# CliMA/CloudMicrophysics.jl

Hardware: AMD Instinct MI355X
Metric: grid-points/sec SB2006 2M tendency sweep (higher is better)
Workload: dtype f32

## Files before the change

cloudmicrophysics.jl_amd/csrc/cmx_sb2006.hpp:

```cpp
#pragma once
#include <cmath>
#include <cstdint>

#include "../../include/cmx.h"
#include "cmx_math.hpp"

namespace cmx {

enum : int { VEL_NONE = 0, VEL_SB = 1, VEL_CHEN = 2, VEL_CHEN_GEN = 3 };

template <typename FT> struct SbConsts {
    FT T_0, LH_v0, dcp, R_v, inv_R_v;
    FT ps_c0, ps_a, ps_b, inv_T_tr;
    FT cp_d, cpm_qt, cpm_ql;
    FT tau_ce;
    FT inv_K, Rv_over_D, eps_1m;
    FT xr_min, xr_max, N0_min, N0_max, lam_min, lam_max, pi_rho_w;
    FT l2_6xstar, l2_Drc;
    FT l2_pi_rho_w, l2_xr_min, l2_xr_max, l2_N0_min, l2_N0_max, l2_lam_min, l2_lam_max, inv_eps_1m;
    FT ga_c1, ga_e1, ga_c2, ga_e2;
    FT gb_c1, gb_e1, gb_c2, gb_e2;
    FT a_vent_1, bSc_vent_1;
    FT sqrt_alpha_nu, beta, ev_rho0_q;
    FT sqrt_alpha_nu_rho0q;
// ... 197 lines not shown
    vt_n = FT(0);
    vt_m = FT(0);
    if constexpr (VEL == VEL_SB) {
        const FT Dr_mean = M::exp2_fin(-l2_lam);
        FT pa0 = FT(1), pb0 = FT(1), pa1 = FT(1), pb1 = FT(1);
        if constexpr (!LIMITED) {
            const FT lam = M::exp2_fin(l2_lam);
            const FT ta = c.rc2 * lam, tb = c.rc2 * (lam + c.cR);
            pa0 = M::exp2_fin(ta * FT(-1.4426950408889634));
            pb0 = pa0 * c.e_rc2cR;
            pa1 = (((ta + FT(3)) * ta + FT(6)) * ta + FT(6)) * pa0 * FT(1.0 / 6.0);
            pb1 = (((tb + FT(3)) * tb + FT(6)) * tb + FT(6)) * pb0 * FT(1.0 / 6.0);
        }
        const FT s = c.vel_s * rs_rho;
        const FT inv_d1 = M::rcp_nz(M::fma(c.cR, Dr_mean, FT(1)));
        const FT inv_d2 = inv_d1 * inv_d1;
        const FT vt0 = M::max(FT(0), s * (c.aR * pa0 - c.bR * pb0 * inv_d1));
        const FT vt1 = M::max(FT(0), s * (c.aR * pa1 - c.bR * pb1 * (inv_d2 * inv_d2)));
        vt_n = no_N_rai ? FT(0) : vt0;
        vt_m = no_q_rai ? FT(0) : vt1;
    } else if constexpr (VEL == VEL_CHEN) {
        const FT lam = M::exp2_fin(l2_lam);
        const FT rho_c = M::max(rho, FT(0));
        const FT t = rho_c - FT(0.5 * kChenGammaRhoMax);
        const FT l2_lam4 = FT(4) * l2_lam;
        FT vt0 = FT(0), vt3 = FT(0);
#pragma unroll
        for (int i = 0; i < 3; ++i) {
            const FT l2_den = M::log2(lam + c.ch_c1000[i]);
            FT L0 = chen_log_eval<S>(c.chl, 0, i, t), L3 = chen_log_eval<S>(c.chl, 1, i, t);
            if (i == 2) { const FT ar = c.ch_a3_pow * M::log2(rho_c); L0 += ar; L3 += ar; }
            const FT e0 = M::exp2(M::fma(-M::fma(-c.ch_b_rho, rho_c, c.chl.b1[i]), l2_den, L0 + l2_lam));
            const FT e3 = M::exp2(M::fma(-M::fma(-c.ch_b_rho, rho_c, c.chl.b4[i]), l2_den, L3 + l2_lam4));
            vt0 = M::fma(c.chl.sgn[i], e0, vt0);
            vt3 = M::fma(c.chl.sgn[i], e3, vt3);
        }
        vt0 = M::max(FT(0), vt0);
        vt3 = M::max(FT(0), vt3);
        {
            const typename M::Mask beyond = rho_c > FT(kChenGammaRhoMax);
            vt0 = beyond ? M::nan() : vt0;
            vt3 = beyond ? M::nan() : vt3;
        }
        vt_n = no_N_rai ? FT(0) : vt0;
        vt_m = no_q_rai ? FT(0) : vt3;
    } else if constexpr (VEL == VEL_CHEN_GEN) {
        const FT lam = M::exp2_fin(l2_lam);
        const FT rho_c = M::max(rho, FT(0));
        const FT l2_q = c.ch_rho0_l2e * rho_c;
        const FT l2_rho = M::log2(rho_c);
        const FT l2_lam_inv = -l2_lam;
        FT vt0 = FT(0), vt3 = FT(0);
#pragma unroll
        for (int i = 0; i < 3; ++i) {
            const FT bi = M::fma(-c.ch_b_rho, rho_c, c.ch_b[i]);
            FT l2_mag = l2_q + bi * c.l2_1000 + (i == 2 ? c.ch_a3_pow * l2_rho : FT(0));
            const FT l2_den = M::log2(lam + c.ch_c1000[i]);
            const FT g1 = tgamma_general<FT>(bi + FT(1));
            const FT e0 = M::exp2(l2_mag - l2_lam_inv - (bi + FT(1)) * l2_den);
            const FT e3 = M::exp2(l2_mag - FT(4) * l2_lam_inv - (bi + FT(4)) * l2_den);
            vt0 = M::fma(c.ch_a[i] * e0, g1, vt0);
            const FT g4 = g1 * (bi + FT(3)) * (bi + FT(2)) * (bi + FT(1)) * FT(1.0 / 6.0);
            vt3 = M::fma(c.ch_a[i] * e3, g4, vt3);
        }
        vt0 = M::max(FT(0), vt0);
        vt3 = M::max(FT(0), vt3);
        vt_n = no_N_rai ? FT(0) : vt0;
        vt_m = no_q_rai ? FT(0) : vt3;
    }
}

template <typename FT, typename CH> inline int chen_vel_kind(const CH &ch) {
    ChenLog<FT> g;
    return make_chen_log<FT>(ch, g) ? VEL_CHEN : VEL_CHEN_GEN;
}

template <typename WR> inline bool sb_integer_exponents(const WR &wr) {
    const auto &sb = wr.seifert_beheng;
    return sb.acnv.b == 3 && sb.accr.c == 4 && sb.self.d == -5;
}
template <typename FT, bool LIMITED, int VEL, bool ICE = false, bool INTPOW = false, typename C>
__device__ __forceinline__ SbRates<FT> sb2006_point(const C &c0, FT rho, FT T, FT q_tot,
                                                    FT q_lcl, FT q_rai, FT N_lcl, FT N_rai,
                                                    FT n_lcl, FT n_rai, FT q_ice = FT(0), FT cpm_qi = FT(0)) {
    using M = Math<FT>;
    const FT eps = FT(M::eps());
    SbRates<FT> r;

    const FT rs_rho = M::rsqrt(rho);
    const FT inv_rho = rs_rho * rs_rho;
    r.inv_rho = inv_rho;

    const C &c = c0;
    const FT inv_T = M::rcp_nz(T);
    const FT L_v = M::fma(c.dcp, T - c.T_0, c.LH_v0);
    const FT l2_ps = M::fma(c.ps_a, M::log2(T * c.inv_T_tr), M::fma(c.ps_b, c.inv_T_tr - inv_T, c.ps_c0));
    const FT p_sat = M::exp2_fin(l2_ps);
    const FT q_liq = q_lcl + q_rai;
    FT q_vap = M::max(FT(0), q_tot - q_liq);
    if constexpr (ICE) q_vap = M::max(FT(0), (q_tot - q_liq) - q_ice);
    const FT rho_RvT = rho * (c.R_v * T);
    const FT inv_p_sat = M::rcp(p_sat);
    const FT inv_RvT = c.inv_R_v * inv_T;
    const FT q_sat = p_sat * (inv_rho * inv_RvT);
    const FT LoRT = L_v * inv_RvT;
    {
        FT cp_air = M::fma(c.cpm_ql, q_liq, M::fma(c.cpm_qt, q_tot, c.cp_d));
        if constexpr (ICE) cp_air = M::fma(cpm_qi, q_ice, cp_air);
        const FT dqsl_dT = q_sat * (LoRT * inv_T - inv_T);
        const FT excess = q_vap - q_sat;
        const FT inv_ts = cp_air * M::rcp_nz(c.tau_ce * M::fma(L_v, dqsl_dT, cp_air));
        const FT evap_lim = -M::min(-excess, M::max(FT(0), q_lcl));
        r.cond = (excess < FT(0) ? evap_lim : excess) * inv_ts;
    }
    const FT S = M::fma(q_vap * rho_RvT, inv_p_sat, FT(-1));
    const FT inv_p_safe = M::min(inv_p_sat, c.inv_eps_1m);
    const FT G = M::rcp_nz(M::fma(L_v * c.inv_K * inv_T, LoRT - FT(1), c.Rv_over_D * T * inv_p_safe));

    const FT sq_lcl = M::max(q_lcl, eps);
    const FT sN_lcl = M::max(N_lcl, eps);
    const FT sq_rai = M::max(q_rai, eps);
    const FT sN_rai = M::max(N_rai, eps);
    const FT L_lcl = rho * sq_lcl;
    const FT L_rai = rho * sq_rai;
    const FT x_lcl_raw = L_lcl * M::rcp_nz(sN_lcl);
    using B = typename M::Mask;
    const B no_q_lcl = q_lcl < eps, no_N_lcl = N_lcl < eps, no_q_rai = q_rai < eps;
    const FT inv_qsum = M::rcp_nz(sq_lcl + sq_rai);
    const FT tau = sq_rai * inv_qsum;
    const FT one_m_tau = sq_lcl * inv_qsum;
    const FT l2_tau = M::log2(tau);
    {
        const C &c = consts_after(c0, G);
        const FT x_lcl = M::min(c.x_star, x_lcl_raw);
        const FT tau_a = M::exp2_fin(c.acnv_a * l2_tau);
        FT pow_b;
        if constexpr (INTPOW) { const FT u = FT(1) - tau_a; pow_b = u * u * u; }
        else pow_b = M::exp2(c.acnv_b * M::log2(FT(1) - tau_a));
        const FT phi_raw = keep(c.acnv_A * tau_a * pow_b);
        const FT phi_au = no_q_rai ? FT(0) : phi_raw;
        const FT u = (L_lcl * x_lcl) * c.sqrt_kfac;
        const FT inv_omt = M::rcp_nz(one_m_tau);
        const FT dL_rai = (u * u) * M::fma(phi_au, inv_omt * inv_omt, FT(1)) * (c.acnv_rho0 * inv_rho);
        const FT dN_rai = dL_rai * c.inv_x_star;
        const B gate = m_or(no_q_lcl, no_N_lcl);
        r.au_dq_rai = gate ? FT(0) : dL_rai * inv_rho;
        r.au_dq_lcl = -r.au_dq_rai;
        r.au_dN_rai = gate ? FT(0) : dN_rai;
        r.au_dN_lcl = FT(-2) * r.au_dN_rai;
    }
    {
        const C &c = consts_after(c0, G);
        const FT Lr = rho * q_lcl;
        const FT sc = -c.ksc * inv_rho * (Lr * Lr) - r.au_dN_lcl;
        r.lsc = no_q_lcl ? FT(0) : sc;
        r.lsc_plus_au = no_q_lcl ? FT(0) : -c.ksc * inv_rho * (Lr * Lr);
    }
    {
        const C &c = consts_after(c0, G);
        FT pow_c;
        if constexpr (INTPOW) { const FT t = tau * M::rcp_nz(tau + c.tau_0), t2 = t * t; pow_c = t2 * t2; }
        else pow_c = M::exp2_fin(c.accr_c * (l2_tau - M::log2(tau + c.tau_0)));
        const FT phi_ac = keep(pow_c);
        const FT k_ac = c.kcr_s * rs_rho * L_rai * phi_ac;
        const FT dq = keep(k_ac * L_lcl * inv_rho);
        const FT dN = keep(-k_ac * sN_lcl);
        const B gate = m_or(no_q_lcl, no_q_rai, no_N_lcl);
        r.ac_dq_rai = gate ? FT(0) : dq;
        r.ac_dq_lcl = -r.ac_dq_rai;
        r.ac_dN_lcl = gate ? FT(0) : dN;
    }

    const C &c_psd = consts_after(c0, r.ac_dN_lcl);
    const SbRainPsd<FT> psd = sb2006_rain_psd<FT, LIMITED>(c_psd, L_rai, sN_rai);
    const FT l2_xr = psd.l2_xr, l2_lam = psd.l2_lam;
    const FT l2_Dr = (l2_xr + c_psd.l2_Drc) * FT(1.0 / 3.0);
    const FT Dr = M::exp2_fin(l2_Dr);
    const B no_N_rai = N_rai < eps;
    {
        const C &c = consts_after(c0, r.ac_dN_lcl);
        FT pw;
        if constexpr (INTPOW) { const FT r1 = M::rcp_nz(M::fma(c.kappa_rr_K, Dr, FT(1))), r2 = r1 * r1; pw = r2 * r2 * r1; }
        else pw = M::exp2_fin(c.self_d * M::log2(M::fma(c.kappa_rr_K, Dr, FT(1))));
        const FT sc = -c.krr_s * rs_rho * N_rai * L_rai * pw;
        const B gate = m_or(no_q_rai, no_N_rai);
        r.rsc = gate ? FT(0) : sc;
        const FT dD = Dr - c.Deq;
        const FT br_lin = keep(c.kbr * dD), br_exp = keep(M::exp2_fin(c.kappa_br_l2e * dD) - FT(1));
        const FT phi_br = (Dr < c.Dr_th) ? FT(-1) : ((Dr <= c.Deq) ? br_lin : br_exp);
        r.rbr = gate ? FT(0) : -(phi_br + FT(1)) * r.rsc;
    }
    {
        const C &c = consts_after(c0, r.rbr);
        const FT l2_t = (c.l2_6xstar - l2_xr) * FT(1.0 / 3.0);
        FT t_star;
        if constexpr (M::IS_F64) t_star = c.tstar_Dr * M::rcp_nz(Dr);
        else t_star = M::exp2_fin(l2_t);
        const FT e_tx = M::exp2_fin(M::fma(t_star, FT(-1.4426950408889634), -l2_xr));
        const FT g_a = M::rcp_nz(M::fma(c.ga_c1, M::exp2_fin(c.ga_e1 * l2_t), c.ga_c2 * M::exp2_fin(c.ga_e2 * l2_t)));
        const FT g_b = M::rcp(M::fma(c.gb_c1, M::exp2_fin(c.gb_e1 * l2_t), c.gb_c2 * M::exp2_fin(c.gb_e2 * l2_t)));
        const FT sqrt_N_Re = c.sqrt_alpha_nu_rho0q * M::sqrt_pos(rs_rho) *
                             M::exp2_fin(FT(0.5) * M::fma(c.beta, l2_xr, l2_Dr));
        const FT Fv0 = M::fma(g_b, sqrt_N_Re, g_a);
        const FT Fv1 = M::fma(c.bSc_vent_1, sqrt_N_Re, c.a_vent_1);
        const FT common = c.two_pi * G * S * N_rai * Dr;
        const FT dN = M::min(FT(0), common * Fv0 * e_tx);
        const FT dq = M::min(FT(0), common * Fv1 * inv_rho);
        const B gate_q = m_or(no_q_rai, N_rai <= eps, S >= FT(0));
        const B gate_N = m_or(gate_q, l2_xr < c.l2_gate_N);
        r.evN = gate_N ? FT(0) : dN;
        r.evq = gate_q ? FT(0) : dq;
    }
    {
        const C &c = consts_after(c0, r.evq);
        const FT tl = no_q_lcl ? FT(0) : clampv(n_lcl, q_lcl * c.inv_xc_max, q_lcl * c.inv_xc_min);
        r.na_lcl = (tl - n_lcl) * c.inv_tau_na;
        const FT tr = no_q_rai ? FT(0) : clampv(n_rai, q_rai * c.inv_xr_max, q_rai * c.inv_xr_min);
        r.na_rai = (tr - n_rai) * c.inv_tau_na;
    }
    sb2006_rain_velocity<FT, LIMITED, VEL>(consts_after(c0, r.evq), rho, rs_rho, l2_lam, no_N_rai, no_q_rai, r.vt_n, r.vt_m);
    return r;
}

}
```

cloudmicrophysics.jl_amd/csrc/cmx_sb2006_kernels.hip:

```cpp
#include <hip/hip_runtime.h>

#include <algorithm>
#include <type_traits>

#include "cmx_sb2006_kernels.hpp"

namespace cmx {

static int decode_vel(uint32_t flags, bool want) {
    if (!want) return VEL_NONE;
    const bool sb = flags & CMX_VEL_SB2006, ch = flags & CMX_VEL_CHEN2022;
    if (sb == ch) return -1;
    return sb ? VEL_SB : VEL_CHEN;
}

#ifndef CMX_TEND_BS
#define CMX_TEND_BS 128
#endif
constexpr int kTendBS = CMX_TEND_BS;

template <typename FT, typename WR, typename TH, typename VL>
static int32_t tendencies_entry(const WR *wr, const TH *tps, const VL *vel, uint32_t flags, int64_t n, const FT *rho,
                                const FT *T, const FT *q_tot, const FT *q_lcl, const FT *n_lcl, const FT *q_rai,
                                const FT *n_rai, FT *dq_lcl, FT *dn_lcl, FT *dq_rai, FT *dn_rai, FT *vt_n, FT *vt_m,
                                void *stream) {
    if (!wr || !tps) return CMX_ERR_BAD_ARG;
    CMX_TRY_COUNT(n);
    if (!rho || !T || !q_tot || !q_lcl || !n_lcl || !q_rai || !n_rai || !dq_lcl || !dn_lcl || !dq_rai || !dn_rai)
        return CMX_ERR_BAD_ARG;
    const bool want_vel = vt_n || vt_m;
    int velk = decode_vel(flags, want_vel);
    if (velk < 0 || (want_vel && !vel)) return CMX_ERR_BAD_ARG;
    if (velk == VEL_CHEN) velk = chen_vel_kind<FT>(vel->chen2022);
    const bool limited = flags & CMX_SB2006_LIMITED;
    if ((flags & CMX_SB2006_LIMITED) && !sb_limiters_ok(*wr)) return CMX_ERR_BAD_ARG;
    if (velk == VEL_SB && !sb_rain_vel_ok(*vel, limited)) return CMX_ERR_BAD_ARG;
    const SbConsts<FT> c = make_sb_consts<FT>(*wr, *tps, vel, (double)Math<FT>::eps_1m());
    const bool intpow = sb_integer_exponents(*wr);
    bool known = true;
    hipStream_t s = reinterpret_cast<hipStream_t>(stream);
    constexpr int VEC = sizeof(FT) == 8 ? 1 : Math<FT>::VEC;
    const void *ptrs[] = {rho, T, q_tot, q_lcl, n_lcl, q_rai, n_rai, dq_lcl, dn_lcl, dq_rai, dn_rai, vt_n, vt_m};
    for_each_range<FT, VEC>(ptrs, n, [&](auto vec_tag, int64_t lo, int64_t count) {
        constexpr int V = decltype(vec_tag)::value;
        SbIn<FT> in{rho + lo, T + lo, q_tot + lo, q_lcl + lo, n_lcl + lo, q_rai + lo, n_rai + lo};
        SbOut<FT> out{dq_lcl + lo, dn_lcl + lo, dq_rai + lo, dn_rai + lo, shift(vt_n, lo), shift(vt_m, lo)};
        const int64_t nvec = count / V;
        known &= dispatch([&](auto L, auto K, auto I) {
            launch<kTendBS>(sb2006_tendencies_kernel<FT, decltype(L)::value, decltype(K)::value, V, kTendBS, 1, true, decltype(I)::value>, nvec, s, c, in, out, nvec);
        }, flag(limited), one_of<VEL_NONE, VEL_SB, VEL_CHEN, VEL_CHEN_GEN>(velk), flag(intpow));
    });
    if (!known) return CMX_ERR_BAD_ARG;
    return launched();
}

template <typename FT, typename WR, typename TH>
static int32_t fields_entry(const WR *wr, const TH *tps, uint32_t flags, int64_t n_seg, int64_t seg_len, const FT *const *in,
                            const int64_t *in_stride, FT *const *out, const int64_t *out_stride, FT *aos, void *stream) {
    if (!wr || !tps || (flags & ~(uint32_t)CMX_SB2006_LIMITED)) return CMX_ERR_BAD_ARG;
    if ((flags & CMX_SB2006_LIMITED) && !sb_limiters_ok(*wr)) return CMX_ERR_BAD_ARG;
    const SbConsts<FT> c = make_sb_consts<FT>(*wr, *tps, (const std::conditional_t<std::is_same_v<FT, float>, cmx_rain_vel_f32, cmx_rain_vel_f64> *)nullptr,
                                              (double)Math<FT>::eps_1m());
    hipStream_t s = reinterpret_cast<hipStream_t>(stream);
    return dispatch_or((int32_t)CMX_ERR_BAD_ARG, [&](auto L, auto I) {
        return launch_layout<FT, Sb2006LayoutPolicy<FT, decltype(L)::value, decltype(I)::value>>(c, n_seg, seg_len, in, in_stride, out, out_stride, aos, s);
    }, flag(flags & CMX_SB2006_LIMITED), flag(sb_integer_exponents(*wr)));
}

template <typename FT, typename WR, typename TH, typename VL>
static int32_t process_entry(const WR *wr, const TH *tps, const VL *vel, uint32_t flags, int64_t n, const FT *q_tot,
                             const FT *q_lcl, const FT *q_rai, const FT *N_lcl, const FT *N_rai, const FT *rho,
                             const FT *T, FT *const out[CMX_SB2006_NPROC], void *stream) {
    if (!wr || !tps || !out) return CMX_ERR_BAD_ARG;
    CMX_TRY_COUNT(n);
    if (!q_tot || !q_lcl || !q_rai || !N_lcl || !N_rai || !rho || !T) return CMX_ERR_BAD_ARG;
    const bool want_vel = out[CMX_SB_RAI_VEL_N] || out[CMX_SB_RAI_VEL_M];
    int velk = decode_vel(flags, want_vel);
    if (velk < 0 || (want_vel && !vel)) return CMX_ERR_BAD_ARG;
    if (velk == VEL_CHEN) velk = chen_vel_kind<FT>(vel->chen2022);
    const bool limited = flags & CMX_SB2006_LIMITED;
    if ((flags & CMX_SB2006_LIMITED) && !sb_limiters_ok(*wr)) return CMX_ERR_BAD_ARG;
    if (velk == VEL_SB && !sb_rain_vel_ok(*vel, limited)) return CMX_ERR_BAD_ARG;
    const SbConsts<FT> c = make_sb_consts<FT>(*wr, *tps, vel, (double)Math<FT>::eps_1m());
    SbProcOut<FT> o;
    for (int k = 0; k < CMX_SB2006_NPROC; ++k) o.col[k] = out[k];
    hipStream_t s = reinterpret_cast<hipStream_t>(stream);
    const dim3 grid(grid_for(n));
    if (!dispatch([&](auto L, auto K) {
            launch_grid(sb2006_process_kernel<FT, decltype(L)::value, decltype(K)::value>, grid, dim3(kBlock), 0, s, c, q_tot, q_lcl, q_rai, N_lcl, N_rai, rho, T, o, n);
        }, flag(limited), one_of<VEL_NONE, VEL_SB, VEL_CHEN, VEL_CHEN_GEN>(velk)))
        return CMX_ERR_BAD_ARG;
    return launched();
}

template <typename FT>
__global__ __launch_bounds__(kBlock) void sb2006_cloud_velocity_kernel(const CloudVelConsts<FT> c, const FT *__restrict__ q_liq,
                                                                       const FT *__restrict__ rho, const FT *__restrict__ N_liq,
                                                                       FT *__restrict__ vt_n, FT *__restrict__ vt_m, const int64_t n) {
    Math<FT>::prepare();
    const int64_t i = (int64_t)blockIdx.x * kBlock + threadIdx.x;
    if (i >= n) return;
    FT v0, v1;
    sb2006_cloud_velocity(c, q_liq[i], rho[i], N_liq[i], v0, v1);
    if (vt_n) vt_n[i] = v0;
    if (vt_m) vt_m[i] = v1;
}

template <typename FT, typename PDF, typename VEL>
static int32_t cloud_velocity_entry(const PDF *pdf, const VEL *vel, int64_t n, const FT *q_liq, const FT *rho, const FT *N_liq, FT *vt_n,
                                    FT *vt_m, void *stream) {
    if (!pdf || !vel) return CMX_ERR_BAD_ARG;
    CMX_TRY_COUNT(n);
    if (!q_liq || !rho || !N_liq) return CMX_ERR_BAD_ARG;
    const CloudVelConsts<FT> c = make_cloud_vel_consts<FT>(*pdf, *vel);
    launch<kBlock>(sb2006_cloud_velocity_kernel<FT>, n, reinterpret_cast<hipStream_t>(stream), c, q_liq, rho, N_liq, vt_n, vt_m, n);
    return launched();
}

template <typename FT> struct Bulk2mConsts {
    uint32_t scheme; FT eps_1m, eps_m;
    FT kk_l2A, kk_a, kk_b, kk_c, kk_accr_A, kk_accr_a, kk_accr_b;
    FT b_l2C, b_a, b_b, b_c, b_N_0, b_d_low, b_d_high, b_k, b_accr_A;
    FT t_a, t_b, t_D, t_thr_c, t_k, t_accr_A;
    FT l_rvol_c, l_E_0, l_R_6C_0, l_k;
};
template <typename FT> __device__ __forceinline__ FT logistic_dev(FT x, FT x_0, FT k, FT eps) {
    using M = Math<FT>;
    x = M::max(FT(0), x);
    const FT xs = M::max(x, eps), x0s = M::max(x_0, eps);
    const FT z = k * (xs * M::rcp(x0s) - x0s * M::rcp(xs));
    const FT r = M::rcp(FT(1) + M::exp2(-z * FT(1.4426950408889634)));
    return x < eps ? FT(0) : (x_0 < eps ? FT(1) : r);
}
template <typename FT>
__global__ __launch_bounds__(kBlock) void bulk_2m_cloud_to_rain_kernel(const Bulk2mConsts<FT> c, const FT *__restrict__ q_lcl,
                                                                       const FT *__restrict__ q_rai, const FT *__restrict__ rho,
                                                                       const FT *__restrict__ N_d, FT *__restrict__ acnv,
                                                                       FT *__restrict__ accr, const int64_t n) {
    Math<FT>::prepare();
    using M = Math<FT>;
    const int64_t i = (int64_t)blockIdx.x * kBlock + threadIdx.x;
    if (i >= n) return;
    const uint32_t sch = c.scheme & 0xffu;
    const bool smooth = c.scheme & CMX_2M_SMOOTH_TRANSITION;
    const FT ql_raw = q_lcl[i], r = rho[i];
    const FT ql = M::max(FT(0), ql_raw);
    if (acnv) {
        const FT Nd = N_d[i];
        const FT l2q = M::log2(ql), l2N = M::log2(Nd), l2r = M::log2(r);
        FT v;
        if (sch == CMX_2M_KK2000) {
            v = M::exp2(c.kk_l2A + c.kk_a * l2q + c.kk_b * l2N + c.kk_c * l2r);
        } else if (sch == CMX_2M_B1994) {
            FT d;
            if (smooth) {
                const FT f = logistic_dev<FT>(Nd, c.b_N_0, c.b_k, c.eps_1m);
                d = f * c.b_d_low + (FT(1) - f) * c.b_d_high;
            } else {
                d = Nd >= c.b_N_0 ? c.b_d_low : c.b_d_high;
            }
            v = M::exp2(c.b_l2C + c.b_a * M::log2(d) + c.b_b * (l2q + l2r) + c.b_c * l2N - l2r);
        } else if (sch == CMX_2M_TC1980) {
            const FT thr = c.t_thr_c * Nd * M::rcp(r);
            const FT out = smooth ? logistic_dev<FT>(ql, thr, c.t_k, c.eps_1m) : (ql - thr > FT(0) ? FT(1) : FT(0));
            v = c.t_D * M::exp2(c.t_a * l2q + c.t_b * l2N) * out;
        } else {
            const FT l2_rv3 = M::log2(c.l_rvol_c * ql_raw * r * M::rcp(Nd));
            const FT r_vol = M::exp2(l2_rv3 * FT(1.0 / 3.0));
            const FT l2_b6 = FT(1.0 / 3.0) * M::log2((r_vol + FT(3)) * M::rcp(r_vol));
            const FT R_6 = M::exp2(l2_b6) * r_vol;
            const FT l2_qr = M::log2(ql_raw * r);
            const FT R_6C = c.l_R_6C_0 * M::exp2(FT(-1.0 / 6.0) * l2_qr) * M::rsqrt(R_6);
            const FT out = smooth ? logistic_dev<FT>(R_6, R_6C, c.l_k, c.eps_1m) : (R_6 - R_6C > FT(0) ? FT(1) : FT(0));
            const FT val = c.l_E_0 * M::exp2(FT(6) * l2_b6 + FT(3) * l2_qr - l2N - l2r) * out;
            v = ql_raw <= c.eps_m ? FT(0) : val;
        }
        acnv[i] = v;
    }
    if (accr) {
        const FT qr = M::max(FT(0), q_rai[i]);
        FT v;
        if (sch == CMX_2M_KK2000) v = c.kk_accr_A * M::exp2(c.kk_accr_a * M::log2(ql * qr) + c.kk_accr_b * M::log2(r));
        else if (sch == CMX_2M_B1994) v = c.b_accr_A * ql * r * qr;
        else v = c.t_accr_A * ql * qr;
        accr[i] = v;
    }
}

template <typename FT, typename SC>
static int32_t bulk_2m_entry(const SC *p, uint32_t scheme, int64_t n, const FT *q_lcl, const FT *q_rai, const FT *rho, const FT *N_d,
                             FT *acnv, FT *accr, void *stream) {
    const uint32_t sch = scheme & 0xffu;
    if (!p || sch > CMX_2M_LD2004 || (scheme & ~(0xffu | CMX_2M_SMOOTH_TRANSITION))) return CMX_ERR_BAD_ARG;
    CMX_TRY_COUNT_LIMIT(n);
    if (sch == CMX_2M_LD2004 && accr) return CMX_ERR_BAD_ARG;
    if (n == 0) return CMX_OK;
    if (!q_lcl || !rho || (acnv && !N_d) || (accr && !q_rai) || (!acnv && !accr)) return CMX_ERR_BAD_ARG;
    const double pi = 3.14159265358979323846;
    Bulk2mConsts<FT> c{};
    c.scheme = scheme; c.eps_1m = Math<FT>::eps_1m(); c.eps_m = Math<FT>::eps();
    c.kk_l2A = (FT)std::log2((double)p->kk2000.acnv_A); c.kk_a = p->kk2000.acnv_a; c.kk_b = p->kk2000.acnv_b; c.kk_c = p->kk2000.acnv_c;
    c.kk_accr_A = p->kk2000.accr_A; c.kk_accr_a = p->kk2000.accr_a; c.kk_accr_b = p->kk2000.accr_b;
    c.b_l2C = (FT)std::log2((double)p->b1994.acnv_C); c.b_a = p->b1994.acnv_a; c.b_b = p->b1994.acnv_b; c.b_c = p->b1994.acnv_c;
    c.b_N_0 = p->b1994.acnv_N_0; c.b_d_low = p->b1994.acnv_d_low; c.b_d_high = p->b1994.acnv_d_high; c.b_k = p->b1994.acnv_k;
    c.b_accr_A = p->b1994.accr_A;
    c.t_a = p->tc1980.acnv_a; c.t_b = p->tc1980.acnv_b; c.t_D = p->tc1980.acnv_D; c.t_k = p->tc1980.acnv_k; c.t_accr_A = p->tc1980.accr_A;
    c.t_thr_c = (FT)((double)p->tc1980.acnv_m0_liq_coeff * std::pow((double)p->tc1980.acnv_r_0, (double)p->tc1980.acnv_me_liq));
    c.l_rvol_c = (FT)(3.0 / 4.0 / pi / (double)p->ld2004.rho_w * 1e18);
    c.l_E_0 = p->ld2004.E_0; c.l_R_6C_0 = p->ld2004.R_6C_0; c.l_k = p->ld2004.k;
    launch<kBlock>(bulk_2m_cloud_to_rain_kernel<FT>, n, reinterpret_cast<hipStream_t>(stream), c, q_lcl, q_rai, rho, N_d, acnv, accr, n);
    return launched();
}

}

extern "C" {

int32_t cmx_bulk_2m_cloud_to_rain_f32(const cmx_bulk_2m_schemes_f32 *schemes, uint32_t scheme, int64_t n, const float *q_lcl,
                                      const float *q_rai, const float *rho, const float *N_d, float *acnv, float *accr, void *stream) {
    return cmx::bulk_2m_entry<float>(schemes, scheme, n, q_lcl, q_rai, rho, N_d, acnv, accr, stream);
}
int32_t cmx_bulk_2m_cloud_to_rain_f64(const cmx_bulk_2m_schemes_f64 *schemes, uint32_t scheme, int64_t n, const double *q_lcl,
                                      const double *q_rai, const double *rho, const double *N_d, double *acnv, double *accr,
                                      void *stream) {
    return cmx::bulk_2m_entry<double>(schemes, scheme, n, q_lcl, q_rai, rho, N_d, acnv, accr, stream);
}

int32_t cmx_sb2006_cloud_terminal_velocity_f32(const cmx_cloud_pdf_sb2006_f32 *pdf_c, const cmx_stokes_vel_f32 *vel, int64_t n,
                                               const float *q_liq, const float *rho, const float *N_liq, float *vt_n, float *vt_m,
                                               void *stream) {
    return cmx::cloud_velocity_entry<float>(pdf_c, vel, n, q_liq, rho, N_liq, vt_n, vt_m, stream);
}
int32_t cmx_sb2006_cloud_terminal_velocity_f64(const cmx_cloud_pdf_sb2006_f64 *pdf_c, const cmx_stokes_vel_f64 *vel, int64_t n,
                                               const double *q_liq, const double *rho, const double *N_liq, double *vt_n, double *vt_m,
                                               void *stream) {
    return cmx::cloud_velocity_entry<double>(pdf_c, vel, n, q_liq, rho, N_liq, vt_n, vt_m, stream);
}

int32_t cmx_sb2006_warm_rain_tendencies_f32(const cmx_warm_rain_2m_f32 *warm_rain, const cmx_thermo_f32 *tps,
                                            const cmx_rain_vel_f32 *vel, uint32_t flags, int64_t n, const float *rho,
                                            const float *T, const float *q_tot, const float *q_lcl, const float *n_lcl,
                                            const float *q_rai, const float *n_rai, float *dq_lcl_dt, float *dn_lcl_dt,
                                            float *dq_rai_dt, float *dn_rai_dt, float *vt_rai_n, float *vt_rai_m,
                                            void *stream) {
    return cmx::tendencies_entry<float>(warm_rain, tps, vel, flags, n, rho, T, q_tot, q_lcl, n_lcl, q_rai, n_rai,
                                        dq_lcl_dt, dn_lcl_dt, dq_rai_dt, dn_rai_dt, vt_rai_n, vt_rai_m, stream);
}

int32_t cmx_sb2006_warm_rain_tendencies_f64(const cmx_warm_rain_2m_f64 *warm_rain, const cmx_thermo_f64 *tps,
                                            const cmx_rain_vel_f64 *vel, uint32_t flags, int64_t n, const double *rho,
                                            const double *T, const double *q_tot, const double *q_lcl,
                                            const double *n_lcl, const double *q_rai, const double *n_rai,
                                            double *dq_lcl_dt, double *dn_lcl_dt, double *dq_rai_dt, double *dn_rai_dt,
                                            double *vt_rai_n, double *vt_rai_m, void *stream) {
    return cmx::tendencies_entry<double>(warm_rain, tps, vel, flags, n, rho, T, q_tot, q_lcl, n_lcl, q_rai, n_rai,
                                         dq_lcl_dt, dn_lcl_dt, dq_rai_dt, dn_rai_dt, vt_rai_n, vt_rai_m, stream);
}

int32_t cmx_sb2006_process_rates_f32(const cmx_warm_rain_2m_f32 *warm_rain, const cmx_thermo_f32 *tps,
                                     const cmx_rain_vel_f32 *vel, uint32_t flags, int64_t n, const float *q_tot,
                                     const float *q_lcl, const float *q_rai, const float *N_lcl, const float *N_rai,
                                     const float *rho, const float *T, float *const out[CMX_SB2006_NPROC],
                                     void *stream) {
    return cmx::process_entry<float>(warm_rain, tps, vel, flags, n, q_tot, q_lcl, q_rai, N_lcl, N_rai, rho, T, out,
                                     stream);
}

int32_t cmx_sb2006_process_rates_f64(const cmx_warm_rain_2m_f64 *warm_rain, const cmx_thermo_f64 *tps,
                                     const cmx_rain_vel_f64 *vel, uint32_t flags, int64_t n, const double *q_tot,
                                     const double *q_lcl, const double *q_rai, const double *N_lcl,
                                     const double *N_rai, const double *rho, const double *T,
                                     double *const out[CMX_SB2006_NPROC], void *stream) {
    return cmx::process_entry<double>(warm_rain, tps, vel, flags, n, q_tot, q_lcl, q_rai, N_lcl, N_rai, rho, T, out,
                                      stream);
}

int32_t cmx_sb2006_warm_rain_tendencies_fields_f32(const cmx_warm_rain_2m_f32 *warm_rain, const cmx_thermo_f32 *tps, uint32_t flags, int64_t n_seg,
                                                   int64_t seg_len, const float *const *in, const int64_t *in_seg_stride, float *const *out,
                                                   const int64_t *out_seg_stride, float *out_aos, void *stream) {
    return cmx::fields_entry<float>(warm_rain, tps, flags, n_seg, seg_len, in, in_seg_stride, out, out_seg_stride, out_aos, stream);
}
int32_t cmx_sb2006_warm_rain_tendencies_fields_f64(const cmx_warm_rain_2m_f64 *warm_rain, const cmx_thermo_f64 *tps, uint32_t flags, int64_t n_seg,
                                                   int64_t seg_len, const double *const *in, const int64_t *in_seg_stride, double *const *out,
                                                   const int64_t *out_seg_stride, double *out_aos, void *stream) {
    return cmx::fields_entry<double>(warm_rain, tps, flags, n_seg, seg_len, in, in_seg_stride, out, out_seg_stride, out_aos, stream);
}

}
```

cloudmicrophysics.jl_amd/csrc/cmx_sb2006_kernels.hpp:

```cpp
#pragma once
#include <hip/hip_runtime.h>

#include "cmx_launch.hpp"
#include "cmx_layout.hpp"
#include "cmx_sb2006.hpp"

namespace cmx {

template <typename FT> struct SbIn { const FT *rho, *T, *q_tot, *q_lcl, *n_lcl, *q_rai, *n_rai; };
template <typename FT> struct SbOut { FT *dq_lcl, *dn_lcl, *dq_rai, *dn_rai, *vt_n, *vt_m; };
template <typename FT> struct SbProcOut { FT *col[CMX_SB2006_NPROC]; };

#ifndef CMX_SB_WAVES
#define CMX_SB_WAVES 1
#endif
template <typename FT, bool LIMITED, int VEL, int VEC, int BS = kBlock, int C = 1, bool NT = true, bool INTPOW = false>
__global__ __launch_bounds__(BS) __attribute__((amdgpu_waves_per_eu((VEL <= VEL_SB && VEC * (int)sizeof(FT) <= 16 && C == 1) ? CMX_SB_WAVES : 1)))
void sb2006_tendencies_kernel(const SbConsts<FT> c, const SbIn<FT> in,
                                                               const SbOut<FT> out, const int64_t nvec) {
    const int64_t base = ((int64_t)blockIdx.x * C) * BS + threadIdx.x;
    FT rho[C][VEC], T[C][VEC], q_tot[C][VEC], q_lcl[C][VEC], n_lcl[C][VEC], q_rai[C][VEC], n_rai[C][VEC];
#pragma unroll
    for (int t = 0; t < C; ++t) {
        const int64_t i = base + (int64_t)t * BS;
        if (i < nvec) {
            load_col<FT, VEC, NT>(in.rho, i, rho[t]);
            load_col<FT, VEC, NT>(in.T, i, T[t]);
            load_col<FT, VEC, NT>(in.q_tot, i, q_tot[t]);
            load_col<FT, VEC, NT>(in.q_lcl, i, q_lcl[t]);
            load_col<FT, VEC, NT>(in.n_lcl, i, n_lcl[t]);
            load_col<FT, VEC, NT>(in.q_rai, i, q_rai[t]);
            load_col<FT, VEC, NT>(in.n_rai, i, n_rai[t]);
        }
    }
    Math<FT>::prepare();
#pragma unroll
    for (int t = 0; t < C; ++t) {
        const int64_t i = base + (int64_t)t * BS;
        if (i >= nvec) continue;
        FT dq_lcl[VEC], dn_lcl[VEC], dq_rai[VEC], dn_rai[VEC], vt_n[VEC], vt_m[VEC];
        constexpr int L = (sizeof(FT) == 4 && VEC % 2 == 0 && VEL == VEL_CHEN) ? 2 : 1;
        if constexpr (L == 1) {
#pragma unroll
            for (int k = 0; k < VEC; ++k) {
                const FT r_ = max0(rho[t][k]);
                const FT qt = max0(q_tot[t][k]);
                const FT ql = max0(q_lcl[t][k]);
                const FT qr = max0(q_rai[t][k]);
                const FT nl = max0(n_lcl[t][k]);
                const FT nr = max0(n_rai[t][k]);
                const bool poisoned = any_nan(rho[t][k], q_tot[t][k], q_lcl[t][k], n_lcl[t][k], q_rai[t][k], n_rai[t][k], T[t][k]);
                const SbRates<FT> p = sb2006_point<FT, LIMITED, VEL, false, INTPOW>(front_consts<FT>(c), r_, T[t][k], qt, ql, qr, r_ * nl, r_ * nr, nl, nr);
                dq_lcl[k] = (p.cond + p.au_dq_lcl) + p.ac_dq_lcl;
                dn_lcl[k] = Math<FT>::fma(p.lsc_plus_au + p.ac_dN_lcl, p.inv_rho, p.na_lcl);
                dq_rai[k] = (p.evq + p.au_dq_rai) + p.ac_dq_rai;
                dn_rai[k] = Math<FT>::fma(((p.evN + p.au_dN_rai) + p.rsc) + p.rbr, p.inv_rho, p.na_rai);
                vt_n[k] = p.vt_n;
                vt_m[k] = p.vt_m;
                const FT poison = poisoned ? Math<FT>::nan() : FT(0);
                dq_lcl[k] += poison; dn_lcl[k] += poison; dq_rai[k] += poison; dn_rai[k] += poison; vt_n[k] += poison; vt_m[k] += poison;
            }
        } else {
            using VT = std::conditional_t<L == 2, f32x2, FT>;
            using MV = Math<VT>;
#pragma unroll
            for (int k = 0; k < VEC; k += L) {
                auto val = [k](const FT (&a)[VEC]) -> VT {
                    if constexpr (L == 2) return VT{a[k], a[k + 1]};
                    else return a[k];
                };
                const VT rho_k = val(rho[t]), T_k = val(T[t]), qt_k = val(q_tot[t]), ql_k = val(q_lcl[t]), nl_k = val(n_lcl[t]), qr_k = val(q_rai[t]), nr_k = val(n_rai[t]);
                const VT r_ = max0(rho_k);
                const VT qt = max0(qt_k);
                const VT ql = max0(ql_k);
                const VT qr = max0(qr_k);
                const VT nl = max0(nl_k);
                const VT nr = max0(nr_k);
                const typename MV::Mask poisoned = nan_mask(rho_k, qt_k, ql_k, nl_k, qr_k, nr_k, T_k);
                const SbRates<VT> p = sb2006_point<VT, LIMITED, VEL, false, INTPOW>(front_consts<FT>(c), r_, T_k, qt, ql, qr, r_ * nl, r_ * nr, nl, nr);
                VT o[6];
                o[0] = (p.cond + p.au_dq_lcl) + p.ac_dq_lcl;
                o[1] = MV::fma(p.lsc_plus_au + p.ac_dN_lcl, p.inv_rho, p.na_lcl);
                o[2] = (p.evq + p.au_dq_rai) + p.ac_dq_rai;
                o[3] = MV::fma(((p.evN + p.au_dN_rai) + p.rsc) + p.rbr, p.inv_rho, p.na_rai);
                o[4] = p.vt_n;
                o[5] = p.vt_m;
                const VT poison = poisoned ? MV::nan() : VT(0);
#pragma unroll
                for (int q = 0; q < 6; ++q) o[q] += poison;
                auto put = [k](FT (&a)[VEC], VT x) {
                    if constexpr (L == 2) { a[k] = x.x; a[k + 1] = x.y; }
                    else a[k] = x;
                };
                put(dq_lcl, o[0]); put(dn_lcl, o[1]); put(dq_rai, o[2]); put(dn_rai, o[3]); put(vt_n, o[4]); put(vt_m, o[5]);
            }
        }
        store_col<FT, VEC, NT>(out.dq_lcl, i, dq_lcl);
        store_col<FT, VEC, NT>(out.dn_lcl, i, dn_lcl);
        store_col<FT, VEC, NT>(out.dq_rai, i, dq_rai);
        store_col<FT, VEC, NT>(out.dn_rai, i, dn_rai);
        if constexpr (VEL != VEL_NONE) {
            if (out.vt_n) store_col<FT, VEC, NT>(out.vt_n, i, vt_n);
            if (out.vt_m) store_col<FT, VEC, NT>(out.vt_m, i, vt_m);
        }
    }
}

template <typename FT, bool LIMITED, bool INTPOW = false> struct Sb2006LayoutPolicy {
    static constexpr int NIN = 7, NOUT = 4, NAOS = 8;
    using Consts = SbConsts<FT>;
    static constexpr bool PACKABLE = true;
    template <typename C, typename VT> static __device__ __forceinline__ void point(const C &c, const VT (&x)[NIN], VT (&y)[NOUT]) {
        using M = Math<VT>;
        const VT r_ = max0(x[0]), qt = max0(x[2]), ql = max0(x[3]);
        const VT nl = max0(x[4]), qr = max0(x[5]), nr = max0(x[6]);
        const SbRates<VT> p = sb2006_point<VT, LIMITED, VEL_NONE, false, INTPOW>(c, r_, x[1], qt, ql, qr, r_ * nl, r_ * nr, nl, nr);
        y[0] = (p.cond + p.au_dq_lcl) + p.ac_dq_lcl;
        y[1] = M::fma(p.lsc_plus_au + p.ac_dN_lcl, p.inv_rho, p.na_lcl);
        y[2] = (p.evq + p.au_dq_rai) + p.ac_dq_rai;
        y[3] = M::fma(((p.evN + p.au_dN_rai) + p.rsc) + p.rbr, p.inv_rho, p.na_rai);
        const VT poison = nan_mask(x[0], x[2], x[3], x[4], x[5], x[6], x[1]) ? M::nan() : VT(0);
        y[0] += poison; y[1] += poison; y[2] += poison; y[3] += poison;
    }
};

template <typename FT, bool LIMITED, int VEL>
__global__ __launch_bounds__(kBlock) void sb2006_process_kernel(const SbConsts<FT> c, const FT *__restrict__ q_tot,
                                                                const FT *__restrict__ q_lcl, const FT *__restrict__ q_rai,
                                                                const FT *__restrict__ N_lcl, const FT *__restrict__ N_rai,
                                                                const FT *__restrict__ rho, const FT *__restrict__ T,
                                                                const SbProcOut<FT> out, const int64_t n) {
    Math<FT>::prepare();
    using M = Math<FT>;
    const int64_t stride = (int64_t)gridDim.x * kBlock;
    for (int64_t i = (int64_t)blockIdx.x * kBlock + threadIdx.x; i < n; i += stride) {
        const FT r_ = rho[i];
        const FT inv_r = M::rcp(r_);
        const SbRates<FT> p = sb2006_point<FT, LIMITED, VEL>(front_consts<FT>(c), r_, T[i], q_tot[i], q_lcl[i], q_rai[i], N_lcl[i],
                                                             N_rai[i], N_lcl[i] * inv_r, N_rai[i] * inv_r);
        const FT poison = any_nan(q_tot[i], q_lcl[i], q_rai[i], N_lcl[i], N_rai[i], r_, T[i]) ? M::nan() : FT(0);
#define CMX_PUT(colid, v) if (out.col[colid]) out.col[colid][i] = (v) + poison
        CMX_PUT(CMX_SB_ACNV_DQ_LCL, p.au_dq_lcl);
        CMX_PUT(CMX_SB_ACNV_DN_LCL, p.au_dN_lcl);
        CMX_PUT(CMX_SB_ACNV_DQ_RAI, p.au_dq_rai);
        CMX_PUT(CMX_SB_ACNV_DN_RAI, p.au_dN_rai);
        CMX_PUT(CMX_SB_LCL_SELFCOL, p.lsc);
        CMX_PUT(CMX_SB_ACCR_DQ_LCL, p.ac_dq_lcl);
        CMX_PUT(CMX_SB_ACCR_DN_LCL, p.ac_dN_lcl);
        CMX_PUT(CMX_SB_ACCR_DQ_RAI, p.ac_dq_rai);
        CMX_PUT(CMX_SB_RAI_SELFCOL, p.rsc);
        CMX_PUT(CMX_SB_RAI_BREAKUP, p.rbr);
        CMX_PUT(CMX_SB_RAI_VEL_N, p.vt_n);
        CMX_PUT(CMX_SB_RAI_VEL_M, p.vt_m);
        CMX_PUT(CMX_SB_EVAP_DN_RAI, p.evN);
        CMX_PUT(CMX_SB_EVAP_DQ_RAI, p.evq);
        CMX_PUT(CMX_SB_NUMADJ_RAI, p.na_rai);
        CMX_PUT(CMX_SB_NUMADJ_LCL, p.na_lcl);
        CMX_PUT(CMX_SB_CONDEVAP, p.cond);
        CMX_PUT(CMX_SB_DEVAP_DN_RAI, N_rai[i] > M::eps() ? p.evN * M::rcp(N_rai[i]) : FT(0));
        CMX_PUT(CMX_SB_DEVAP_DQ_RAI, q_rai[i] > M::eps() ? p.evq * M::rcp(q_rai[i]) : FT(0));
#undef CMX_PUT
    }
}

}
```

Measured before the change: 116.1 billion.

## Add compile-time-constant SB2006 tendency kernel for default parameter set

Adds a float32 tendency kernel that uses a constexpr table of the default folded SB2006 constants, instead of passing them as a kernel argument. The host takes this kernel only when every runtime constant matches the table bit for bit and integer exponents apply; otherwise it uses the generic kernel. The aim is to let the compiler fold literals and simplify arithmetic, and to cut scalar constant loads, with an occupancy hint of four waves per EU. In exchange it adds a host-side comparison on each call, an environment-variable opt-out and duplicated constants that must stay in sync.

```diff
diff --git a/cloudmicrophysics.jl_amd/csrc/cmx_sb2006.hpp b/cloudmicrophysics.jl_amd/csrc/cmx_sb2006.hpp
--- a/cloudmicrophysics.jl_amd/csrc/cmx_sb2006.hpp
+++ b/cloudmicrophysics.jl_amd/csrc/cmx_sb2006.hpp
@@ -373,9 +373,9 @@
     {
         const C &c = consts_after(c0, G);
         const FT Lr = rho * q_lcl;
-        const FT sc = -c.ksc * inv_rho * (Lr * Lr) - r.au_dN_lcl;
+        const FT sc = -(c.ksc * inv_rho * (Lr * Lr)) - r.au_dN_lcl;
         r.lsc = no_q_lcl ? FT(0) : sc;
-        r.lsc_plus_au = no_q_lcl ? FT(0) : -c.ksc * inv_rho * (Lr * Lr);
+        r.lsc_plus_au = no_q_lcl ? FT(0) : -(c.ksc * inv_rho * (Lr * Lr));
     }
     {
         const C &c = consts_after(c0, G);
diff --git a/cloudmicrophysics.jl_amd/csrc/cmx_sb2006_default_consts.inc b/cloudmicrophysics.jl_amd/csrc/cmx_sb2006_default_consts.inc
--- /dev/null
+++ b/cloudmicrophysics.jl_amd/csrc/cmx_sb2006_default_consts.inc
@@ -0,0 +1,79 @@
+CMX_SBD(T_0, 0x1.1128f6p+8f)
+CMX_SBD(LH_v0, 0x1.3146p+21f)
+CMX_SBD(dcp, -0x1.224p+11f)
+CMX_SBD(R_v, 0x1.cd8p+8f)
+CMX_SBD(inv_R_v, 0x1.1c0354p-9f)
+CMX_SBD(ps_c0, 0x1.2835e6p+3f)
+CMX_SBD(ps_a, -0x1.4202c6p+2f)
+CMX_SBD(ps_b, 0x1.324486p+13f)
+CMX_SBD(inv_T_tr, 0x1.dfd604p-9f)
+CMX_SBD(cp_d, 0x1.f64p+9f)
+CMX_SBD(cpm_qt, 0x1.ab4p+9f)
+CMX_SBD(cpm_ql, 0x1.224p+11f)
+CMX_SBD(tau_ce, 0x1.4p+3f)
+CMX_SBD(inv_K, 0x1.4d5556p+5f)
+CMX_SBD(Rv_over_D, 0x1.379702p+24f)
+CMX_SBD(eps_1m, 0x1p-42f)
+CMX_SBD(xr_min, 0x1.1ddf7ep-32f)
+CMX_SBD(xr_max, 0x1.4f8b58p-18f)
+CMX_SBD(pi_rho_w, 0x1.88b2f8p+11f)
+CMX_SBD(l2_6xstar, -0x1.d417c8p+4f)
+CMX_SBD(l2_Drc, -0x1.2108cp+3f)
+CMX_SBD(l2_pi_rho_w, 0x1.73c0c2p+3f)
+CMX_SBD(l2_xr_min, -0x1.fd73cap+4f)
+CMX_SBD(l2_xr_max, -0x1.19c116p+4f)
+CMX_SBD(inv_eps_1m, 0x1p+42f)
+CMX_SBD(ga_c1, 0x1.99851ep-2f)
+CMX_SBD(ga_e1, 0x1.028f5cp+0f)
+CMX_SBD(ga_c2, 0x1.1e4432p-1f)
+CMX_SBD(ga_e2, 0x1.ccccccp+0f)
+CMX_SBD(gb_c1, 0x1.833748p-1f)
+CMX_SBD(gb_e1, 0x1.643568p-3f)
+CMX_SBD(gb_c2, 0x1.462ab8p+1f)
+CMX_SBD(gb_e2, 0x1.cd4fep-1f)
+CMX_SBD(a_vent_1, 0x1.b78d74p-2f)
+CMX_SBD(bSc_vent_1, 0x1.4a2edp-3f)
+CMX_SBD(sqrt_alpha_nu, 0x1.8a0c2ap+11f)
+CMX_SBD(beta, 0x1.10624ep-2f)
+CMX_SBD(ev_rho0_q, 0x1.0d52c6p+0f)
+CMX_SBD(sqrt_alpha_nu_rho0q, 0x1.9e8e3p+11f)
+CMX_SBD(two_pi, 0x1.921fb6p+2f)
+CMX_SBD(l2_gate_N, -0x1.b6b9e6p+5f)
+CMX_SBD(tstar_Dr, 0x1.2dc462p-13f)
+CMX_SBD(sqrt_kfac, 0x1.aa9fdp+30f)
+CMX_SBD(x_star, 0x1.1ddf7ep-32f)
+CMX_SBD(inv_x_star, 0x1.ca7f4ep+31f)
+CMX_SBD(acnv_A, 0x1.9p+8f)
+CMX_SBD(acnv_a, 0x1.666666p-1f)
+CMX_SBD(acnv_b, 0x1.8p+1f)
+CMX_SBD(acnv_rho0, 0x1.39999ap+0f)
+CMX_SBD(ksc, 0x1.e648d6p+32f)
+CMX_SBD(kcr_s, 0x1.73e244p+2f)
+CMX_SBD(tau_0, 0x1.a36e2ep-15f)
+CMX_SBD(accr_c, 0x1p+2f)
+CMX_SBD(krr_s, 0x1.f85868p+2f)
+CMX_SBD(kappa_rr_K, 0x1.0d3d2ap+8f)
+CMX_SBD(self_d, -0x1.4p+2f)
+CMX_SBD(Deq, 0x1.d7dbf4p-11f)
+CMX_SBD(Dr_th, 0x1.6f0068p-12f)
+CMX_SBD(kbr, 0x1.f4p+9f)
+CMX_SBD(kappa_br_l2e, 0x1.9ec65ap+11f)
+CMX_SBD(inv_tau_na, 0x1.47ae14p-7f)
+CMX_SBD(inv_xc_min, 0x1.b117bcp+47f)
+CMX_SBD(inv_xc_max, 0x1.ca7f4ep+31f)
+CMX_SBD(inv_xr_min, 0x1.ca7f4ep+31f)
+CMX_SBD(inv_xr_max, 0x1.86ap+17f)
+CMX_SBD(N0_min, 0x1.e848p+17f)
+CMX_SBD(N0_max, 0x1.312dp+24f)
+CMX_SBD(lam_min, 0x1.f4p+9f)
+CMX_SBD(lam_max, 0x1.388p+13f)
+CMX_SBD(l2_N0_min, 0x1.1ee7b4p+4f)
+CMX_SBD(l2_N0_max, 0x1.840e52p+4f)
+CMX_SBD(l2_lam_min, 0x1.3ee7b4p+3f)
+CMX_SBD(l2_lam_max, 0x1.a934fp+3f)
+CMX_SBD(vel_s, 0x1.1b571p+0f)
+CMX_SBD(aR, 0x1.34ccccp+3f)
+CMX_SBD(bR, 0x1.49999ap+3f)
+CMX_SBD(cR, 0x1.2cp+9f)
+CMX_SBD(rc2, 0x1.c7aef6p-14f)
+CMX_SBD(e_rc2cR, 0x1.dfb076p-1f)
diff --git a/cloudmicrophysics.jl_amd/csrc/cmx_sb2006_kernels.hip b/cloudmicrophysics.jl_amd/csrc/cmx_sb2006_kernels.hip
--- a/cloudmicrophysics.jl_amd/csrc/cmx_sb2006_kernels.hip
+++ b/cloudmicrophysics.jl_amd/csrc/cmx_sb2006_kernels.hip
@@ -1,6 +1,8 @@
 #include <hip/hip_runtime.h>
 
 #include <algorithm>
+#include <cstdlib>
+#include <cstring>
 #include <type_traits>
 
 #include "cmx_sb2006_kernels.hpp"
@@ -18,6 +20,28 @@
 #define CMX_TEND_BS 128
 #endif
 constexpr int kTendBS = CMX_TEND_BS;
+
+static uint32_t f32_bits(float x) {
+    uint32_t u;
+    std::memcpy(&u, &x, sizeof u);
+    return u;
+}
+static bool sb_consts_are_default(const SbConsts<float> &c, bool limited, int velk) {
+    bool same = true;
+#define CMX_SAME(m) same &= f32_bits(c.m) == f32_bits(SbDefaultConstsF32::m);
+    CMX_SB_FOLDED_CORE(CMX_SAME)
+    if (limited) { CMX_SB_FOLDED_LIM(CMX_SAME) }
+    if (velk == VEL_SB) { CMX_SB_FOLDED_VEL(CMX_SAME) }
+#undef CMX_SAME
+    return same;
+}
+static bool sb_takes_default_kernel(const SbConsts<float> &c, bool limited, int velk, bool intpow) {
+    if (!intpow || (velk != VEL_NONE && velk != VEL_SB)) return false;
+    const char *env = std::getenv("CMX_SB2006_DEFAULT_KERNEL");
+    if (env && env[0] == '0' && env[1] == 0) return false;
+    return sb_consts_are_default(c, limited, velk);
+}
+static bool sb_takes_default_kernel(const SbConsts<double> &, bool, int, bool) { return false; }
 
 template <typename FT, typename WR, typename TH, typename VL>
 static int32_t tendencies_entry(const WR *wr, const TH *tps, const VL *vel, uint32_t flags, int64_t n, const FT *rho,
@@ -37,6 +61,7 @@
     if (velk == VEL_SB && !sb_rain_vel_ok(*vel, limited)) return CMX_ERR_BAD_ARG;
     const SbConsts<FT> c = make_sb_consts<FT>(*wr, *tps, vel, (double)Math<FT>::eps_1m());
     const bool intpow = sb_integer_exponents(*wr);
+    const bool defaults = sb_takes_default_kernel(c, limited, velk, intpow);
     bool known = true;
     hipStream_t s = reinterpret_cast<hipStream_t>(stream);
     constexpr int VEC = sizeof(FT) == 8 ? 1 : Math<FT>::VEC;
@@ -46,6 +71,14 @@
         SbIn<FT> in{rho + lo, T + lo, q_tot + lo, q_lcl + lo, n_lcl + lo, q_rai + lo, n_rai + lo};
         SbOut<FT> out{dq_lcl + lo, dn_lcl + lo, dq_rai + lo, dn_rai + lo, shift(vt_n, lo), shift(vt_m, lo)};
         const int64_t nvec = count / V;
+        if constexpr (std::is_same_v<FT, float> && V == 4) {
+            if (defaults) {
+                known &= dispatch([&](auto L, auto K) {
+                    launch<kSbDefaultBS>(sb2006_tendencies_default_kernel<decltype(L)::value, decltype(K)::value>, nvec, s, in, out, nvec);
+                }, flag(limited), one_of<VEL_NONE, VEL_SB>(velk));
+                return;
+            }
+        }
         known &= dispatch([&](auto L, auto K, auto I) {
             launch<kTendBS>(sb2006_tendencies_kernel<FT, decltype(L)::value, decltype(K)::value, V, kTendBS, 1, true, decltype(I)::value>, nvec, s, c, in, out, nvec);
         }, flag(limited), one_of<VEL_NONE, VEL_SB, VEL_CHEN, VEL_CHEN_GEN>(velk), flag(intpow));
@@ -247,6 +280,27 @@
                                         dq_lcl_dt, dn_lcl_dt, dq_rai_dt, dn_rai_dt, vt_rai_n, vt_rai_m, stream);
 }
 
+int32_t cmxdiag_sb2006_consts_f32(const cmx_warm_rain_2m_f32 *warm_rain, const cmx_thermo_f32 *tps, const cmx_rain_vel_f32 *vel, float *out, int32_t cap) {
+    if (!warm_rain || !tps || (cap > 0 && !out)) return CMX_ERR_BAD_ARG;
+    const cmx::SbConsts<float> c = cmx::make_sb_consts<float>(*warm_rain, *tps, vel, (double)cmx::Math<float>::eps_1m());
+    int32_t k = 0;
+#define CMX_PUT(m) { if (k < cap) out[k] = c.m; ++k; }
+    CMX_SB_FOLDED_CORE(CMX_PUT)
+    CMX_SB_FOLDED_LIM(CMX_PUT)
+    CMX_SB_FOLDED_VEL(CMX_PUT)
+#undef CMX_PUT
+    return k;
+}
+int32_t cmxdiag_sb2006_variant_f32(const cmx_warm_rain_2m_f32 *warm_rain, const cmx_thermo_f32 *tps, const cmx_rain_vel_f32 *vel, uint32_t flags) {
+    using namespace cmx;
+    if (!warm_rain || !tps) return 0;
+    const int velk = decode_vel(flags, vel != nullptr);
+    const bool limited = flags & CMX_SB2006_LIMITED;
+    if (velk < 0 || (limited && !sb_limiters_ok(*warm_rain)) || (velk == VEL_SB && !sb_rain_vel_ok(*vel, limited))) return 0;
+    const SbConsts<float> c = make_sb_consts<float>(*warm_rain, *tps, vel, (double)Math<float>::eps_1m());
+    return sb_takes_default_kernel(c, limited, velk, sb_integer_exponents(*warm_rain)) ? 1 : 0;
+}
+
 int32_t cmx_sb2006_warm_rain_tendencies_f64(const cmx_warm_rain_2m_f64 *warm_rain, const cmx_thermo_f64 *tps,
                                             const cmx_rain_vel_f64 *vel, uint32_t flags, int64_t n, const double *rho,
                                             const double *T, const double *q_tot, const double *q_lcl,
diff --git a/cloudmicrophysics.jl_amd/csrc/cmx_sb2006_kernels.hpp b/cloudmicrophysics.jl_amd/csrc/cmx_sb2006_kernels.hpp
--- a/cloudmicrophysics.jl_amd/csrc/cmx_sb2006_kernels.hpp
+++ b/cloudmicrophysics.jl_amd/csrc/cmx_sb2006_kernels.hpp
@@ -14,10 +14,8 @@
 #ifndef CMX_SB_WAVES
 #define CMX_SB_WAVES 1
 #endif
-template <typename FT, bool LIMITED, int VEL, int VEC, int BS = kBlock, int C = 1, bool NT = true, bool INTPOW = false>
-__global__ __launch_bounds__(BS) __attribute__((amdgpu_waves_per_eu((VEL <= VEL_SB && VEC * (int)sizeof(FT) <= 16 && C == 1) ? CMX_SB_WAVES : 1)))
-void sb2006_tendencies_kernel(const SbConsts<FT> c, const SbIn<FT> in,
-                                                               const SbOut<FT> out, const int64_t nvec) {
+template <typename FT, bool LIMITED, int VEL, int VEC, int BS, int C, bool NT, bool INTPOW, typename CT>
+__device__ __forceinline__ void sb2006_tendencies_body(const CT &c, const SbIn<FT> &in, const SbOut<FT> &out, const int64_t nvec) {
     const int64_t base = ((int64_t)blockIdx.x * C) * BS + threadIdx.x;
     FT rho[C][VEC], T[C][VEC], q_tot[C][VEC], q_lcl[C][VEC], n_lcl[C][VEC], q_rai[C][VEC], n_rai[C][VEC];
 #pragma unroll
@@ -104,6 +102,45 @@
             if (out.vt_m) store_col<FT, VEC, NT>(out.vt_m, i, vt_m);
         }
     }
+}
+
+template <typename FT, bool LIMITED, int VEL, int VEC, int BS = kBlock, int C = 1, bool NT = true, bool INTPOW = false>
+__global__ __launch_bounds__(BS) __attribute__((amdgpu_waves_per_eu((VEL <= VEL_SB && VEC * (int)sizeof(FT) <= 16 && C == 1) ? CMX_SB_WAVES : 1)))
+void sb2006_tendencies_kernel(const SbConsts<FT> c, const SbIn<FT> in,
+                                                               const SbOut<FT> out, const int64_t nvec) {
+    sb2006_tendencies_body<FT, LIMITED, VEL, VEC, BS, C, NT, INTPOW>(c, in, out, nvec);
+}
+
+#define CMX_SB_FOLDED_CORE(X)                                                                                                                       \
+    X(T_0) X(LH_v0) X(dcp) X(R_v) X(inv_R_v) X(ps_c0) X(ps_a) X(ps_b) X(inv_T_tr) X(cp_d) X(cpm_qt) X(cpm_ql) X(tau_ce) X(inv_K) X(Rv_over_D)      \
+    X(eps_1m) X(xr_min) X(xr_max) X(pi_rho_w) X(l2_6xstar) X(l2_Drc) X(l2_pi_rho_w) X(l2_xr_min) X(l2_xr_max) X(inv_eps_1m) X(ga_c1) X(ga_e1)      \
+    X(ga_c2) X(ga_e2) X(gb_c1) X(gb_e1) X(gb_c2) X(gb_e2) X(a_vent_1) X(bSc_vent_1) X(sqrt_alpha_nu) X(beta) X(ev_rho0_q) X(sqrt_alpha_nu_rho0q)   \
+    X(two_pi) X(l2_gate_N) X(tstar_Dr) X(sqrt_kfac) X(x_star) X(inv_x_star) X(acnv_A) X(acnv_a) X(acnv_b) X(acnv_rho0) X(ksc) X(kcr_s) X(tau_0)    \
+    X(accr_c) X(krr_s) X(kappa_rr_K) X(self_d) X(Deq) X(Dr_th) X(kbr) X(kappa_br_l2e) X(inv_tau_na) X(inv_xc_min) X(inv_xc_max) X(inv_xr_min)      \
+    X(inv_xr_max)
+#define CMX_SB_FOLDED_LIM(X) X(N0_min) X(N0_max) X(lam_min) X(lam_max) X(l2_N0_min) X(l2_N0_max) X(l2_lam_min) X(l2_lam_max)
+#define CMX_SB_FOLDED_VEL(X) X(vel_s) X(aR) X(bR) X(cR) X(rc2) X(e_rc2cR)
+
+struct SbDefaultConstsF32 {
+#define CMX_SBD(name, value) static constexpr float name = value;
+#include "cmx_sb2006_default_consts.inc"
+#undef CMX_SBD
+};
+
+#ifndef CMX_SBD_WAVES
+#define CMX_SBD_WAVES 4
+#endif
+#if CMX_SBD_WAVES > 1
+#define CMX_SBD_WAVES_ATTR __attribute__((amdgpu_waves_per_eu(CMX_SBD_WAVES, CMX_SBD_WAVES)))
+#else
+#define CMX_SBD_WAVES_ATTR
+#endif
+constexpr int kSbDefaultBS = 128;
+template <bool LIMITED, int VEL>
+__global__ __launch_bounds__(kSbDefaultBS) CMX_SBD_WAVES_ATTR
+void sb2006_tendencies_default_kernel(const SbIn<float> in, const SbOut<float> out, const int64_t nvec) {
+    static_assert(VEL == VEL_NONE || VEL == VEL_SB, "the table holds no Chen-2022 constants");
+    sb2006_tendencies_body<float, LIMITED, VEL, 4, kSbDefaultBS, 1, true, true>(SbDefaultConstsF32{}, in, out, nvec);
 }
 
 template <typename FT, bool LIMITED, bool INTPOW = false> struct Sb2006LayoutPolicy {
```

After: 115.9 billion. No clear change (-0.2%).
